# AdrianPerezHerrero/HDP-GPC

Measured on AMD Instinct MI355X. Metric: GP log-lik evals/sec (NxK batch, T-point segments), higher is better.
Workload: dtype f64; 1 GPU; BASELINE configs[1]: synthetic 2048 segments x 8 clusters, T=128, fp64, irregular segment grids (per-pair Gram + Cholesky + score); segments=2048, segments_per_gpu=2048, clusters=8, T=128

## Files before the change

hdpgpc_amd/csrc/hgp_pairs_acc.hip:

```cpp
#include <hip/hip_runtime.h>
#include <math.h>
#include <stdint.h>

#include "hgp_internal.hpp"
#include "tile_f64.hpp"

using namespace hgp;

namespace {

__host__ __device__ constexpr int ntl(int NB) { return NB * (NB - 1) / 2; }
__host__ __device__ constexpr int tl(int K, int Kp) { return K * (K - 1) / 2 + Kp; }

__global__ void k_acc_flags(double* scal, int K, double tol, int32_t* acc_list) {
  if (threadIdx.x != 0 || blockIdx.x != 0) return;
  int n = 0;
  for (int k = 0; k < K; ++k) {
    const double ck = scal[8 * k] * scal[8 * k + 6];
    const double bound = F64_EPS * ck * ck;
    const bool flag = (tol == 0.0) || (tol > 0.0 && !(bound <= tol));
    scal[8 * k + 7] = flag ? 1.0 : 0.0;
    if (flag) acc_list[1 + n++] = k;
  }
  acc_list[0] = n;
}

template <int NB>
__global__ __launch_bounds__(64) void k_acc_factor(double* A, int TP, const double* scal, int32_t* info) {
  __shared__ __attribute__((aligned(16))) double scr[DIAG_SCR];
  const int k = blockIdx.x, lane = threadIdx.x;
  if (scal[8 * k + 7] == 0.0) return;
  double* Ak = A + (size_t)k * TP * TP;
  d4 U[NB * (NB + 1) / 2];
  d4 R[NB];
  load_upper_only<NB>(U, Ak, TP, TP, lane);
  PivotAcc pa;
  pa.init();
  wave_factor<NB, 0>(U, R, scr, nullptr, nullptr, lane, pa, Ak, TP, TP);
  if (lane == 0 && info && pa.info != 0) info[k] = pa.info;
}

struct AccPrepArgs {
  const double* L;
  const double* S;
  const double* mean;
  const double* scal;
  int T, TP, NB;
  double* Lop;
  double* LTop;
  double* Dop;
  double* Sop;
  double* mu;
};

__global__ __launch_bounds__(256) void k_acc_prep(AccPrepArgs a) {
  const int k = blockIdx.x;
  if (a.scal[8 * k + 7] == 0.0) return;
  const int lane = threadIdx.x & 63, g = lane >> 4, c = lane & 15;
  const int wv = blockIdx.y * 4 + (threadIdx.x >> 6), nwv = gridDim.y * 4;
  const int NB = a.NB, TP = a.TP;
  const double* L = a.L + (size_t)k * TP * TP;
  const double* S = a.S + (size_t)k * TP * TP;
  const int nl = ntl(NB);
  double* Lop = a.Lop + (size_t)k * nl * 256;
  double* LTop = a.LTop + (size_t)k * nl * 256;
  double* Dop = a.Dop + (size_t)k * 4 * NB * 256;
  double* Sop = a.Sop + (size_t)k * NB * NB * 256;
  if (blockIdx.y == 0)
    for (int i = threadIdx.x; i < TP; i += 256) a.mu[(size_t)k * TP + i] = (i < a.T) ? a.mean[(size_t)k * a.T + i] : 0.0;
  const int items = nl + NB + NB * NB;
  for (int it = wv; it < items; it += nwv) {
    if (it < nl) {
      int Kb = 1;
      while (tl(Kb + 1, 0) <= it) ++Kb;
      const int Kp = it - tl(Kb, 0);
      d4 lo, lt;
#pragma unroll
      for (int s = 0; s < 4; ++s) {
        lo[s] = L[(size_t)(16 * Kb + c) * TP + 16 * Kp + 4 * s + g];
        lt[s] = L[(size_t)(16 * Kb + 4 * s + g) * TP + 16 * Kp + c];
      }
      *reinterpret_cast<d4*>(Lop + ((size_t)it * 64 + lane) * 4) = lo;
      *reinterpret_cast<d4*>(LTop + ((size_t)it * 64 + lane) * 4) = lt;
    } else if (it < nl + NB) {
      const int Kb = it - nl;
      const double* D = L + (size_t)(16 * Kb) * TP + 16 * Kb;
      d4 a1, a2, a1t, a2t;
#pragma unroll
      for (int r = 0; r < 4; ++r) {
        const double* B = D + (size_t)(4 * r) * TP + 4 * r;
        const double l00 = B[0], l10 = B[TP], l11 = B[TP + 1], l20 = B[2 * TP], l21 = B[2 * TP + 1], l22 = B[2 * TP + 2],
                     l30 = B[3 * (size_t)TP], l31 = B[3 * (size_t)TP + 1], l32 = B[3 * (size_t)TP + 2], l33 = B[3 * (size_t)TP + 3];
        double w[4][4];
#pragma unroll
        for (int i = 0; i < 4; ++i)
#pragma unroll
          for (int j = 0; j < 4; ++j) w[i][j] = 0.0;
        const double r0 = 1.0 / l00, r1 = 1.0 / l11, r2 = 1.0 / l22, r3 = 1.0 / l33;
        w[0][0] = r0;
        w[1][0] = -(l10 * w[0][0]) * r1;
        w[2][0] = -(l20 * w[0][0] + l21 * w[1][0]) * r2;
        w[3][0] = -(l30 * w[0][0] + l31 * w[1][0] + l32 * w[2][0]) * r3;
        w[1][1] = r1;
        w[2][1] = -(l21 * w[1][1]) * r2;
        w[3][1] = -(l31 * w[1][1] + l32 * w[2][1]) * r3;
        w[2][2] = r2;
        w[3][2] = -(l32 * w[2][2]) * r3;
        w[3][3] = r3;
        const int ci = c & 3;
        double wf = 0.0, wt = 0.0;
#pragma unroll
        for (int i = 0; i < 4; ++i)
#pragma unroll
          for (int j = 0; j < 4; ++j) {
            if (i == ci && j == g) wf = w[i][j];
            if (i == g && j == ci) wt = w[i][j];
          }
        const bool mine = (c >> 2) == r;
        a1[r] = mine ? wf : 0.0;
        a1t[r] = mine ? wt : 0.0;
        a2[r] = (c >= 4 * r + 4) ? D[(size_t)c * TP + 4 * r + g] : 0.0;
        a2t[r] = (c < 4 * r) ? D[(size_t)(4 * r + g) * TP + c] : 0.0;
      }
      *reinterpret_cast<d4*>(Dop + ((size_t)(0 * NB + Kb) * 64 + lane) * 4) = a1;
      *reinterpret_cast<d4*>(Dop + ((size_t)(1 * NB + Kb) * 64 + lane) * 4) = a2;
      *reinterpret_cast<d4*>(Dop + ((size_t)(2 * NB + Kb) * 64 + lane) * 4) = a1t;
      *reinterpret_cast<d4*>(Dop + ((size_t)(3 * NB + Kb) * 64 + lane) * 4) = a2t;
    } else {
      const int t = it - nl - NB, Kb = t / NB, Kp = t % NB;
      d4 so;
#pragma unroll
      for (int s = 0; s < 4; ++s) so[s] = S[(size_t)(16 * Kp + 4 * s + g) * TP + 16 * Kb + c];
      *reinterpret_cast<d4*>(Sop + ((size_t)t * 64 + lane) * 4) = so;
    }
  }
}

struct AccArgs {
  const double* x;
  const double* y;
  int N, Ts;
  const double* xb;
  int T;
  const double* scal;
  const double* mu;
  const double* Lop;
  const double* LTop;
  const double* Dop;
  const double* Sop;
  const int32_t* acc_list;
  const double* first_noise;
  const int32_t* sel;
  int K;
  double* out_quad;
  double* out_logdet;
  int32_t* out_info;
  double* sscr;
  double score_add;
  int score_on;
};

template <int NB>
struct AccLds {
  static constexpr int TP = 16 * NB;
  static constexpr size_t DOUBLES = (size_t)NB * 256  + 256  + 5 * TP  + DIAG_SCR + 32;
  static constexpr size_t BYTES = DOUBLES * sizeof(double) + 16 * sizeof(int);
};

__device__ __forceinline__ d4 ld4(const double* base, unsigned off) { return *reinterpret_cast<const d4*>(base + off); }

template <int NB>
__global__ __launch_bounds__(64 * CoopH<NB>::NW, (NB <= 8) ? 2 : 1) void k_pairs_acc(AccArgs a) {
  using H = CoopH<NB>;
  constexpr int NW = H::NW, TP = 16 * NB;
  extern __shared__ __attribute__((aligned(16))) double smem[];
  double* rowbuf = smem;
  double* Wbuf = rowbuf + NB * 256;
  double* dvec = Wbuf + 256;
  double* xs = dvec + TP;
  double* ys = xs + TP;
  double* xbs = ys + TP;
  double* mus = xbs + TP;
  double* scr = mus + TP;
  double* red = scr + DIAG_SCR;
  int* redi = reinterpret_cast<int*>(red + 32);
  const int tid = threadIdx.x, lane = tid & 63, g = lane >> 4, c = lane & 15;
  const int wave = __builtin_amdgcn_readfirstlane(tid >> 6);
  const int T = a.T, Ts = a.Ts;
  const int nflag = a.acc_list[0];
  if (nflag == 0) return;
  const long npairs = a.sel ? (long)a.N : (long)a.N * nflag;
  double* Ssc = a.sscr + (size_t)blockIdx.x * NB * NB * 256;

  for (long p = blockIdx.x; p < npairs; p += gridDim.x) {
    int n, kc;
    if (a.sel) {
      n = (int)p;
      kc = a.sel[n];
      if (a.scal[8 * kc + 7] == 0.0) continue;
    } else {
      n = (int)(p / nflag);
      kc = a.acc_list[1 + (int)(p % nflag)];
    }
    kc = __builtin_amdgcn_readfirstlane(kc);
    const double* sc = a.scal + 8 * kc;
    const double cc = sc[0], ell = sc[1], noise = sc[2];
    const bool iso = sc[3] != 0.0;
    const size_t oidx = a.sel ? (size_t)n : (size_t)n * a.K + kc;
    const double fn = a.first_noise ? a.first_noise[oidx] : 0.0;
    __syncthreads();
    for (int i = tid; i < TP; i += 64 * NW) {
      xs[i] = (i < Ts) ? a.x[(size_t)n * Ts + i] / ell : 1e150 * (double)(1 + i);
      ys[i] = (i < Ts) ? a.y[(size_t)n * Ts + i] : 0.0;
      xbs[i] = (i < T) ? a.xb[i] / ell : -1e150 * (double)(1 + i);
      mus[i] = a.mu[(size_t)kc * TP + i];
    }
    __syncthreads();
    const double* Lop = a.Lop + (size_t)kc * ntl(NB) * 256;
    const double* LTop = a.LTop + (size_t)kc * ntl(NB) * 256;
    const double* Dop = a.Dop + (size_t)kc * 4 * NB * 256;
    const double* Sop = a.Sop + (size_t)kc * NB * NB * 256;
    double* Sl = Ssc;

    double dsq = 0.0;
#pragma unroll
    for (int q = 0; q < 2; ++q) {
      const int J = (q == 0) ? wave : NB - 1 - wave;
      d4 X[NB];
#pragma unroll
      for (int K = 0; K < NB; ++K) {
        const unsigned l4 = (unsigned)launder(lane) * 4u;
        {
          const int ln = launder(lane);
          const double xj = xs[16 * J + (ln & 15)];
#pragma unroll
          for (int r = 0; r < 4; ++r) {
            const double u = xbs[16 * K + 4 * r + (ln >> 4)] - xj;
            X[K][r] = cc * exp(-0.5 * (u * u));
          }
        }
#pragma unroll
        for (int Kp = 0; Kp < K; ++Kp) {
          const d4 lo = ld4(Lop + tl(K, Kp) * 256, l4);
#pragma unroll
          for (int s = 0; s < 4; ++s) X[K] = mfma_sub(lo[s], X[Kp][s], X[K]);
        }
        const d4 a1 = ld4(Dop + (0 * NB + K) * 256, l4), a2 = ld4(Dop + (1 * NB + K) * 256, l4);
#pragma unroll
        for (int r = 0; r < 4; ++r) {
          d4 t = X[K];
          t[r] = 0.0;
          t = mfma(a1[r], X[K][r], t);
          X[K] = (r < 3) ? mfma_sub(a2[r], t[r], t) : t;
        }
      }
#pragma unroll
      for (int K = NB - 1; K >= 0; --K) {
        const unsigned l4 = (unsigned)launder(lane) * 4u;
#pragma unroll
        for (int Kp = NB - 1; Kp > K; --Kp) {
          const d4 lt = ld4(LTop + tl(Kp, K) * 256, l4);
#pragma unroll
          for (int s = 0; s < 4; ++s) X[K] = mfma_sub(lt[s], X[Kp][s], X[K]);
        }
        const d4 a1 = ld4(Dop + (2 * NB + K) * 256, l4), a2 = ld4(Dop + (3 * NB + K) * 256, l4);
#pragma unroll
        for (int r = 3; r >= 0; --r) {
          d4 t = X[K];
          t[r] = 0.0;
          t = mfma(a1[r], X[K][r], t);
          X[K] = (r > 0) ? mfma_sub(a2[r], t[r], t) : t;
        }
      }
      double pj = 0.0;
#pragma unroll
      for (int K = 0; K < NB; ++K) {
        const int ln = launder(lane);
        const unsigned l4 = (unsigned)ln * 4u;
#pragma unroll
        for (int r = 0; r < 4; ++r) pj = fma(X[K][r], mus[16 * K + 4 * r + (ln >> 4)], pj);
        *reinterpret_cast<d4*>(Sl + (K * NB + J) * 256 + l4) = X[K];
      }
      pj = xrow_sum(pj);
      if (g == 0) {
        const int j = 16 * J + c;
        const double d = ys[j] - pj;
        dvec[j] = d;
        dsq = fma(d, d, dsq);
      }
    }
    __syncthreads();

    if (iso) {
      dsq = wave_sum(dsq);
      if (lane == 0) red[wave] = dsq;
      __syncthreads();
      if (tid == 0) {
        const double v = sc[4] + fn;
        const double v2 = v + 1e-8 * fmax(fabs(v), F64_EPS);
        double tot_ = 0.0;
        for (int w_ = 0; w_ < NW; ++w_) tot_ += red[w_];
        a.out_quad[oidx] = a.score_on ? fma(-0.5, tot_ / v2, a.score_add) : (tot_ / v2);
        if (a.out_logdet) a.out_logdet[oidx] = (double)Ts * log(v2);
        if (a.out_info) a.out_info[oidx] = (v2 > 0.0) ? 0 : 1;
      }
      continue;
    }

    d4 U[H::NT];
#pragma unroll
    for (int q = 0; q < 2; ++q) {
      const int J = (q == 0) ? wave : NB - 1 - wave;
      const double xj = xs[16 * J + c];
#pragma unroll
      for (int I = 0; I < (q == 0 ? NW : NB); ++I) {
        const int ln = launder(lane);
        d4 kt = (d4){0.0, 0.0, 0.0, 0.0};
        if (I <= J) {
#pragma unroll
          for (int r = 0; r < 4; ++r) {
            const double u = xs[16 * I + (ln >> 4) + 4 * r] - xs[16 * J + (ln & 15)];
            kt[r] = cc * exp(-0.5 * (u * u));
          }
          if (I == J) {
#pragma unroll
            for (int r = 0; r < 4; ++r)
              if ((ln >> 4) + 4 * r == (ln & 15)) kt[r] = (16 * I + (ln & 15) < Ts) ? cc + noise : 1.0;
          }
          U[q == 0 ? H::slotA(I) : H::slotB(I)] = kt;
        }
      }
#pragma nounroll
      for (int K = 0; K < NB; ++K) {
        const unsigned l4 = (unsigned)launder(lane) * 4u;
        d4 Q;
#pragma unroll
        for (int r = 0; r < 4; ++r) {
          const double u = xbs[16 * K + 4 * r + g] - xj;
          Q[r] = -(cc * exp(-0.5 * (u * u)));
        }
#pragma unroll
        for (int Kp = 0; Kp < NB; ++Kp) {
          const d4 so = ld4(Sop + (K * NB + Kp) * 256, l4);
          const d4 sb = ld4(Sl + (Kp * NB + J) * 256, l4);
#pragma unroll
          for (int s = 0; s < 4; ++s) Q = mfma(so[s], sb[s], Q);
        }
#pragma unroll
        for (int I = 0; I < (q == 0 ? NW : NB); ++I) {
          if (I <= J) {
            const d4 sa = ld4(Sl + (K * NB + I) * 256, l4);
#pragma unroll
            for (int s = 0; s < 4; ++s)
              U[q == 0 ? H::slotA(I) : H::slotB(I)] = mfma(sa[s], Q[s], U[q == 0 ? H::slotA(I) : H::slotB(I)]);
          }
        }
      }
    }

    {
      const double sh = 1e-6 + fn;
      const double dm = cooph_diag_abs_mean<NB>(U, Ts, wave, lane, sh, red);
      cooph_add_diag<NB>(U, sh + 1e-8 * fmax(dm, F64_EPS), Ts, wave, lane);
    }
    PivotAcc pa;
    pa.init();
    double zq = cooph_factor<NB>(U, rowbuf, Wbuf, scr, wave, lane, pa, Ts, dvec);
    int info;
    const double ld = cooph_logdet_info<NB>(pa, wave, lane, red, redi, info);
    zq = wave_sum(zq);
    if (lane == 0) red[8 + wave] = zq;
    __syncthreads();
    if (tid == 0) {
      double tot_ = 0.0;
      for (int w_ = 0; w_ < NW; ++w_) tot_ += red[8 + w_];
      a.out_quad[oidx] = a.score_on ? fma(-0.5, tot_, a.score_add) : (tot_);
      if (a.out_logdet) a.out_logdet[oidx] = ld;
      if (a.out_info) a.out_info[oidx] = info;
    }
  }
}

template <int NB>
int launch_pairs_acc(const AccArgs& a, hipStream_t st) {
  const size_t lds = AccLds<NB>::BYTES;
  hipLaunchKernelGGL(k_pairs_acc<NB>, dim3(acc_grid_for(NB)), dim3(64 * CoopH<NB>::NW), lds, st, a);
  return launch_status();
}

}

size_t hgp_internal_acc_bytes(int TP, int K, size_t* sizes) {
  const int NB = TP / 16;
  size_t s[6];
  s[0] = (size_t)K * ntl(NB) * 256 * sizeof(double);
  s[1] = s[0];
  s[2] = (size_t)K * 4 * NB * 256 * sizeof(double);
  s[3] = (size_t)K * NB * NB * 256 * sizeof(double);
  s[4] = (size_t)K * TP * sizeof(double);
  s[5] = (size_t)acc_grid_for(NB) * NB * NB * 256 * sizeof(double);
  size_t tot = 0;
  for (int i = 0; i < 6; ++i) {
    if (sizes) sizes[i] = s[i];
    tot += (s[i] + 255) & ~(size_t)255;
  }
  return tot;
}

int hgp_internal_acc_prep(hgp_pairs_plan* p, const double* mean, hipStream_t st) {
  const int K = p->K, TP = p->TP, NB = p->NB;
  hipLaunchKernelGGL(k_acc_flags, dim3(1), dim3(64), 0, st, p->d_scal, K, p->acc_tol, p->d_acc_list);
  if (p->acc_tol < 0.0) return launch_status();
  if (NB <= 8)
    dispatch_nb_wave(TP, [&](auto nb) {
      hipLaunchKernelGGL(k_acc_factor<decltype(nb)::value>, dim3(K), dim3(64), 0, st, p->d_A, TP, p->d_scal, (int32_t*)nullptr);
    });
  AccPrepArgs a{p->d_A, p->d_S, mean, p->d_scal, p->T, TP, NB, p->d_Lop, p->d_LTop, p->d_Dop, p->d_Sop, p->d_mu};
  hipLaunchKernelGGL(k_acc_prep, dim3(K, 8), dim3(256), 0, st, a);
  return launch_status();
}

int hgp_internal_pairs_acc(const hgp_pairs_plan* p, const double* x, const double* y, int N, int Ts, const double* first_noise,
                           const int32_t* sel, double* out_quad, double* out_logdet, int32_t* out_info, hipStream_t st) {
  if (p->acc_tol < 0.0) return 0;
  AccArgs a{x, y, N, Ts, p->d_xb, p->T, p->d_scal, p->d_mu, p->d_Lop, p->d_LTop, p->d_Dop, p->d_Sop, p->d_acc_list,
            first_noise, sel, p->K, out_quad, out_logdet, out_info, p->d_sscr, -0.5 * (double)Ts * 1.8378770664093453, p->score_out};
  return dispatch_nb(p->NB, [&](auto nb) { return launch_pairs_acc<decltype(nb)::value>(a, st); });
}
```

hdpgpc_amd/csrc/hgp_plan.hip:

```cpp
#include <algorithm>
#include <new>

#include "hgp_internal.hpp"
#include "tile_f64.hpp"

using namespace hgp;

namespace {

struct PrepArgs {
  const double* xb;
  const double* mean;
  const double* Sigma;
  int T, TP, K;
  const double* theta;
  double* scal;
  double* A;
  double* S;
  double* xb_copy;
};

__global__ __launch_bounds__(256) void k_prep_build(PrepArgs a) {
  __shared__ double red[256];
  __shared__ int redi[256];
  const int k = blockIdx.x, tid = threadIdx.x;
  const int T = a.T, TP = a.TP;
  const double* Sg = a.Sigma + (size_t)k * T * T;
  const double c = a.theta[3 * k], ell = a.theta[3 * k + 1], noise = a.theta[3 * k + 2];
  double s_abs = 0.0, s_sgn = 0.0;
  for (int i = tid; i < T; i += 256) {
    double d = Sg[(size_t)i * T + i];
    s_abs += fabs(d);
    s_sgn += d;
  }
  red[tid] = s_abs;
  __syncthreads();
  for (int o = 128; o > 0; o >>= 1) {
    if (tid < o) red[tid] += red[tid + o];
    __syncthreads();
  }
  const double mean_abs = red[0] / T;
  __syncthreads();
  red[tid] = s_sgn;
  __syncthreads();
  for (int o = 128; o > 0; o >>= 1) {
    if (tid < o) red[tid] += red[tid + o];
    __syncthreads();
  }
  const double mS = red[0] / T;
  int bad = 0;
  for (int i = tid; i < T; i += 256) {
    double d = Sg[(size_t)i * T + i];
    if (!(fabs(d - mS) <= 1e-8 + 1e-5 * fabs(mS))) bad = 1;
  }
  redi[tid] = bad;
  __syncthreads();
  for (int o = 128; o > 0; o >>= 1) {
    if (tid < o) redi[tid] |= redi[tid + o];
    __syncthreads();
  }
  const double jit = 1e-4 * fmax(mean_abs, F64_EPS);
  if (tid == 0 && blockIdx.y == 0) {
    double* sc = a.scal + 8 * k;
    sc[0] = c;
    sc[1] = ell;
    sc[2] = noise;
    sc[3] = redi[0] ? 0.0 : 1.0;
    sc[4] = mS;
    sc[5] = jit;
    sc[6] = 0.0;
  }
  if (k == 0 && blockIdx.y == 0)
    for (int i = tid; i < TP; i += 256) a.xb_copy[i] = (i < T) ? a.xb[i] : 0.0;
  double* Ak = a.A + (size_t)k * TP * TP;
  double* Sk = a.S + (size_t)k * TP * TP;
  for (int idx = blockIdx.y * 256 + tid; idx < TP * TP; idx += gridDim.y * 256) {
    int i = idx / TP, j = idx % TP;
    double av, sv = 0.0;
    if (i < T && j < T) {
      double u = a.xb[i] / ell - a.xb[j] / ell;
      av = c * exp(-0.5 * (u * u));
      if (i == j) av += jit;
      sv = 0.5 * (Sg[(size_t)i * T + j] + Sg[(size_t)j * T + i]);
    } else {
      av = (i == j) ? 1.0 : 0.0;
    }
    Ak[idx] = av;
    Sk[idx] = sv;
  }
}

struct PrepFinalArgs {
  const double* Q;
  const double* Kinv;
  const double* mean;
  double* scal;
  int T, TP;
  double* Mp;
  double* ap;
  int interleave;
  int32_t* fb;
};

__global__ __launch_bounds__(256) void k_prep_final(PrepFinalArgs a) {
  const int k = blockIdx.x, tid = threadIdx.x;
  if (a.fb && k == 0 && blockIdx.y == 0 && tid == 0) {
    a.fb[0] = 0;
    a.fb[1 + PAIRS_FB_CAP] = 0;
  }
  const int T = a.T, TP = a.TP;
  const double c = a.scal[8 * k];
  const double* Q = a.Q + (size_t)k * TP * TP;
  const double* Ki = a.Kinv + (size_t)k * TP * TP;
  double* Mp = a.Mp + (size_t)k * TP * TP;
  __shared__ double tq[32][33], tk[32][33];
  const int NHh = (TP / 16) / 2, nt = TP / 32;
  const int tx = tid & 31, ty = tid >> 5;
  for (int t = blockIdx.y; t < nt * nt; t += gridDim.y) {
    const int bi = t / nt, bj = t % nt;
    __syncthreads();
#pragma unroll
    for (int r = 0; r < 4; ++r) {
      const int y = ty + 8 * r;
      tq[y][tx] = Q[(size_t)(32 * bj + y) * TP + 32 * bi + tx];
      tk[y][tx] = Ki[(size_t)(32 * bj + y) * TP + 32 * bi + tx];
    }
    __syncthreads();
#pragma unroll
    for (int r = 0; r < 4; ++r) {
      const int y = ty + 8 * r;
      const int i = 32 * bi + y, j = 32 * bj + tx;
      double v = 0.0;
      if (i < T && j < T)
        v = (c * c) * (0.5 * (Q[(size_t)i * TP + j] + tq[tx][y]) - 0.5 * (Ki[(size_t)i * TP + j] + tk[tx][y]));
      int jp = j;
      if (a.interleave) {
        const int hh = j / (16 * NHh), tl = (j / 16) % NHh, cc = j % 16;
        const int loc = (tl < 2 * (NHh / 2)) ? 32 * (tl / 2) + 2 * cc + (tl & 1) : 16 * (NHh - 1) + cc;
        jp = 16 * NHh * hh + loc;
      }
      Mp[(size_t)i * TP + jp] = v;
    }
  }
  const double* mu = a.mean + (size_t)k * T;
  __shared__ double red[256];
  double rmax = 0.0;
  for (int i = blockIdx.y * 256 + tid; i < TP; i += gridDim.y * 256) {
    double s = 0.0, rs = 0.0;
    if (i < T) {
#pragma unroll 8
      for (int j = 0; j < T; ++j) {
        const double kij = Ki[(size_t)j * TP + i];
        s = fma(kij, mu[j], s);
        rs += fabs(kij);
      }
    }
    a.ap[(size_t)k * TP + i] = c * s;
    rmax = fmax(rmax, rs);
  }
  red[tid] = rmax;
  __syncthreads();
  for (int o = 128; o > 0; o >>= 1) {
    if (tid < o) red[tid] = fmax(red[tid], red[tid + o]);
    __syncthreads();
  }
  if (tid == 0) atomicMax(reinterpret_cast<unsigned long long*>(a.scal + 8 * k + 6), (unsigned long long)__double_as_longlong(red[0]));
}

static int tp_for(int n) {
  if (n <= HGP_MAX_T_WAVE) return 16 * nb_for(n);
  return n <= 192 ? 192 : 256;
}

size_t plan_layout(hgp_pairs_plan* p, int T, int Ts_max, int K, char* base) {
  const size_t TP = (size_t)tp_for(std::max(T, Ts_max));
  const size_t mat = (size_t)K * TP * TP * sizeof(double);
  p->TP = (int)TP;
  p->NB = p->TP / 16;
  p->coop = p->TP > HGP_MAX_T_WAVE;
  size_t o = 0;
  auto take = [&](auto*& member, size_t bytes) {
    if (base) member = reinterpret_cast<std::remove_reference_t<decltype(member)>>(base + o);
    o += (bytes + 255) & ~(size_t)255;
  };
  take(p->d_theta, (size_t)K * 3 * sizeof(double));
  take(p->d_scal, (size_t)K * 8 * sizeof(double));
  take(p->d_A, mat);
  take(p->d_S, mat);
  take(p->d_Z, mat);
  take(p->d_Kinv, mat);
  take(p->d_P, mat);
  take(p->d_Q, mat);
  take(p->d_Mp, mat);
  take(p->d_ap, (size_t)K * TP * sizeof(double));
  take(p->d_perm, (size_t)K * sizeof(int32_t));
  take(p->d_xb, TP * sizeof(double));
  if (p->coop) {
    const size_t nb = (size_t)p->NB;
    const size_t cap = (nb >= 12) ? 48 : (nb == 8 ? 24 : 16);
    const size_t over = nb * nb > cap ? nb * nb - cap : 0;
    p->nscr = over ? (nb >= 12 ? 512 : 1024) : 0;
    p->escr_stride = (long)(over * 256);
    take(p->d_escr, (size_t)p->nscr * over * 256 * sizeof(double));
    take(p->d_eflags, ((size_t)p->nscr + 1) * sizeof(int32_t));
  }
  size_t sz[6];
  hgp_internal_acc_bytes((int)TP, K, sz);
  take(p->d_Lop, sz[0]);
  take(p->d_LTop, sz[1]);
  take(p->d_Dop, sz[2]);
  take(p->d_Sop, sz[3]);
  take(p->d_mu, sz[4]);
  take(p->d_sscr, sz[5]);
  take(p->d_acc_list, (size_t)(K + 1) * sizeof(int32_t));
  take(p->d_fb, (size_t)(PAIRS_FB_CAP + 2) * sizeof(int32_t));
  return o;
}

}

#ifdef HGP_STAMPS
unsigned long long* hgp_internal_stamp_dev = nullptr;
#endif

extern "C" {

size_t hgp_pairs_plan_device_bytes(int T, int Ts_max, int K) {
  if (T <= 0 || Ts_max <= 0 || K <= 0) return 0;
  hgp_pairs_plan sizing;
  return plan_layout(&sizing, T, Ts_max, K, nullptr);
}

int hgp_pairs_plan_create(hgp_pairs_plan** plan, int T, int Ts_max, int K, const double* theta_host, void* dev_buf,
                          size_t dev_bytes) {
  if (!plan || !theta_host || !dev_buf || T <= 0 || Ts_max <= 0 || K <= 0) return -1;
  if (T > HGP_MAX_T_COOP || Ts_max > HGP_MAX_T_COOP) return -2;
  if (dev_bytes < hgp_pairs_plan_device_bytes(T, Ts_max, K)) return -1;
  for (int k = 0; k < K; ++k)
    if (!(theta_host[3 * k] > 0.0) || !(theta_host[3 * k + 1] > 0.0)) return -1;
  hgp_pairs_plan* p = new (std::nothrow) hgp_pairs_plan();
  if (!p) return -1;
  p->T = T;
  p->K = K;
  p->theta.assign(theta_host, theta_host + 3 * (size_t)K);
  p->perm.resize(K);
  for (int k = 0; k < K; ++k) p->perm[k] = k;
  std::stable_sort(p->perm.begin(), p->perm.end(),
                   [&](int a, int b) { return p->theta[3 * a + 1] < p->theta[3 * b + 1]; });
  for (int i = 0; i < K;) {
    int j = i;
    double ell = p->theta[3 * p->perm[i] + 1];
    while (j < K && p->theta[3 * p->perm[j] + 1] == ell) ++j;
    p->grp_beg.push_back(i);
    p->grp_end.push_back(j);
    p->grp_ell.push_back(ell);
    i = j;
  }
  plan_layout(p, T, Ts_max, K, (char*)dev_buf);
  if (hipMemset(p->d_fb, 0, (size_t)(PAIRS_FB_CAP + 2) * sizeof(int32_t)) != hipSuccess) {
    delete p;
    return 1000 + (int)hipGetLastError();
  }
  if (p->coop && hipMemset(p->d_eflags, 0, (p->nscr + 1) * sizeof(int32_t)) != hipSuccess) {
    delete p;
    return 1000 + (int)hipGetLastError();
  }
  if (hipMemcpy(p->d_theta, p->theta.data(), sizeof(double) * 3 * K, hipMemcpyHostToDevice) != hipSuccess ||
      hipMemcpy(p->d_perm, p->perm.data(), sizeof(int32_t) * K, hipMemcpyHostToDevice) != hipSuccess) {
    delete p;
    return 1000 + (int)hipGetLastError();
  }
  *plan = p;
  return 0;
}

void hgp_pairs_plan_destroy(hgp_pairs_plan* plan) { delete plan; }

const double* hgp_pairs_plan_scalars(const hgp_pairs_plan* plan) { return plan ? plan->d_scal : nullptr; }

int hgp_pairs_plan_update(hgp_pairs_plan* p, const double* x_basis, const double* mean, const double* Sigma,
                          int32_t* info, void* stream) {
  if (!p || !x_basis || !mean || !Sigma) return -1;
  hipStream_t st = (hipStream_t)stream;
  const int K = p->K, T = p->T, TP = p->TP;
  PrepArgs pa{x_basis, mean, Sigma, T, TP, K, p->d_theta, p->d_scal, p->d_A, p->d_S, p->d_xb};
  hipLaunchKernelGGL(k_prep_build, dim3(K, 8), dim3(256), 0, st, pa);
  PotrfArgs fa{p->d_A, TP, K, 0.0, 0.0, p->d_Z, nullptr, info};
  fa.inv_info = 1;
  fa.symmetric = 1;
  if (int rc = hgp_internal_chol_inverse(fa, p->NB, st)) return rc;
  const long sm = (long)TP * TP;
  GemmArgs g1{p->d_Z, p->d_Z, p->d_Kinv, TP, TP, TP, TP, TP, TP, sm, sm, sm, 1.0, 0.0, 1, 0};
  GemmArgs g2{p->d_S, p->d_Kinv, p->d_P, TP, TP, TP, TP, TP, TP, sm, sm, sm, 1.0, 0.0, 0, 0};
  GemmArgs g3{p->d_Kinv, p->d_P, p->d_Q, TP, TP, TP, TP, TP, TP, sm, sm, sm, 1.0, 0.0, 0, 0};
  hgp_internal_gemm(g1, K, st);
  hgp_internal_gemm(g2, K, st);
  hgp_internal_gemm(g3, K, st);
  PrepFinalArgs fin{p->d_Q, p->d_Kinv, mean, p->d_scal, T, TP, p->d_Mp, p->d_ap, p->coop ? 0 : 1, p->d_fb};
  hipLaunchKernelGGL(k_prep_final, dim3(K, 8), dim3(256), 0, st, fin);
  if (p->d_eflags && p->nscr > 0 && hipMemsetAsync(p->d_eflags, 0, (p->nscr + 1) * sizeof(int32_t), st) != hipSuccess) return launch_status();
  int rc = hgp_internal_acc_prep(p, mean, st);
  return rc ? rc : launch_status();
}

int hgp_pairs_plan_set_accuracy(hgp_pairs_plan* p, double tol) {
  if (!p || tol != tol) return -1;
  p->acc_tol = tol;
  return 0;
}

int hgp_pairs_plan_set_score_output(hgp_pairs_plan* p, int on) {
  if (!p) return -1;
  p->score_out = on ? 1 : 0;
  return 0;
}

int hgp_loglik_pairs_f64(const hgp_pairs_plan* p, const double* x, const double* y, int N, int Ts,
                         const double* first_noise, const int32_t* sel, double* out_quad, double* out_logdet,
                         int32_t* out_info, void* stream) {
  if (N == 0) return 0;
  if (!p || !x || !y || !out_quad || N < 0 || Ts <= 0) return -1;
  if (Ts > HGP_MAX_T_COOP) return -2;
  if (Ts > p->TP) return -2;
  hipStream_t st = (hipStream_t)stream;
  int rc = 0;
  if (p->coop && p->d_eflags && p->nscr > 0 &&
      hipMemsetAsync(p->d_eflags, 0, (p->nscr + 1) * sizeof(int32_t), st) != hipSuccess)
    return launch_status();
  for (size_t gi = 0; gi < p->grp_beg.size() && rc == 0; ++gi) {
    PairsArgs a{x, y, N, Ts, p->d_xb, p->T, p->d_Mp, p->d_ap, p->d_scal, p->d_perm, p->grp_beg[gi], p->grp_end[gi],
                p->grp_ell[gi], first_noise, sel,
#ifdef HGP_STAMPS
                hgp_internal_stamp_dev,
#endif
                p->K, out_quad, out_logdet, out_info, p->d_escr, p->d_eflags, p->nscr, p->escr_stride,
                env_on("HGP_PAIRS_GENERIC") ? 1 : 0, -0.5 * (double)Ts * 1.8378770664093453, p->score_out, p->d_fb};
    rc = hgp_internal_pairs_fast(a, p->NB, p->coop, st);
  }
  if (rc == 0) rc = hgp_internal_pairs_acc(p, x, y, N, Ts, first_noise, sel, out_quad, out_logdet, out_info, st);
  return rc;
}

#ifdef HGP_STAMPS
int hgp_debug_stamps(unsigned long long* out8_host) {
  if (!hgp_internal_stamp_dev) {
    if (hipMalloc(&hgp_internal_stamp_dev, 128) != hipSuccess) return 1;
    (void)hipMemset(hgp_internal_stamp_dev, 0, 128);
  }
  if (hipMemcpy(out8_host, hgp_internal_stamp_dev, 128, hipMemcpyDeviceToHost) != hipSuccess) return 1;
  (void)hipMemset(hgp_internal_stamp_dev, 0, 128);
  return 0;
}
#endif

}
```

Before: 15.43 million evals/s.

## Fuse plan-update GEMMs and accuracy setup into fewer custom kernels

Replaces the two generic batched GEMMs (S·Kinv, Kinv·P) and the final M'/a' kernel with two templated MFMA tile kernels for the non-cooperative path. These compute P, then Q tiles with the symmetrised M' and interleaved column layout, and fold the a' reduction into the first kernel. The accuracy flag, Cholesky factor and operand packing are merged into a single setup kernel. Gram/Sigma construction is retiled over a 3-D grid. The aim is fewer kernel launches and fewer global round-trips during plan updates, at the cost of more specialised code paths and intra-block fences that the correctness of the fused factor-then-pack step relies on.

Result: no change. 15.57 million evals/s (median of 6 runs) (+0.9%).

```diff
diff --git a/hdpgpc_amd/csrc/hgp_pairs_acc.hip b/hdpgpc_amd/csrc/hgp_pairs_acc.hip
--- a/hdpgpc_amd/csrc/hgp_pairs_acc.hip
+++ b/hdpgpc_amd/csrc/hgp_pairs_acc.hip
@@ -12,32 +12,25 @@
 __host__ __device__ constexpr int ntl(int NB) { return NB * (NB - 1) / 2; }
 __host__ __device__ constexpr int tl(int K, int Kp) { return K * (K - 1) / 2 + Kp; }
 
+__device__ __forceinline__ bool acc_flag_of(const double* scal, int k, double tol) {
+  const double ck = scal[8 * k] * scal[8 * k + 6];
+  const double bound = F64_EPS * ck * ck;
+  return (tol == 0.0) || (tol > 0.0 && !(bound <= tol));
+}
+
+__device__ __forceinline__ void acc_write_flags(double* scal, int K, double tol, int32_t* acc_list) {
+  int n = 0;
+  for (int k = 0; k < K; ++k) {
+    const bool flag = acc_flag_of(scal, k, tol);
+    scal[8 * k + 7] = flag ? 1.0 : 0.0;
+    if (flag) acc_list[1 + n++] = k;
+  }
+  acc_list[0] = n;
+}
+
 __global__ void k_acc_flags(double* scal, int K, double tol, int32_t* acc_list) {
   if (threadIdx.x != 0 || blockIdx.x != 0) return;
-  int n = 0;
-  for (int k = 0; k < K; ++k) {
-    const double ck = scal[8 * k] * scal[8 * k + 6];
-    const double bound = F64_EPS * ck * ck;
-    const bool flag = (tol == 0.0) || (tol > 0.0 && !(bound <= tol));
-    scal[8 * k + 7] = flag ? 1.0 : 0.0;
-    if (flag) acc_list[1 + n++] = k;
-  }
-  acc_list[0] = n;
-}
-
-template <int NB>
-__global__ __launch_bounds__(64) void k_acc_factor(double* A, int TP, const double* scal, int32_t* info) {
-  __shared__ __attribute__((aligned(16))) double scr[DIAG_SCR];
-  const int k = blockIdx.x, lane = threadIdx.x;
-  if (scal[8 * k + 7] == 0.0) return;
-  double* Ak = A + (size_t)k * TP * TP;
-  d4 U[NB * (NB + 1) / 2];
-  d4 R[NB];
-  load_upper_only<NB>(U, Ak, TP, TP, lane);
-  PivotAcc pa;
-  pa.init();
-  wave_factor<NB, 0>(U, R, scr, nullptr, nullptr, lane, pa, Ak, TP, TP);
-  if (lane == 0 && info && pa.info != 0) info[k] = pa.info;
+  acc_write_flags(scal, K, tol, acc_list);
 }
 
 struct AccPrepArgs {
@@ -53,11 +46,8 @@
   double* mu;
 };
 
-__global__ __launch_bounds__(256) void k_acc_prep(AccPrepArgs a) {
-  const int k = blockIdx.x;
-  if (a.scal[8 * k + 7] == 0.0) return;
+__device__ __forceinline__ void acc_pack(const AccPrepArgs& a, int k, int it0, int it1, int wv, int nwv) {
   const int lane = threadIdx.x & 63, g = lane >> 4, c = lane & 15;
-  const int wv = blockIdx.y * 4 + (threadIdx.x >> 6), nwv = gridDim.y * 4;
   const int NB = a.NB, TP = a.TP;
   const double* L = a.L + (size_t)k * TP * TP;
   const double* S = a.S + (size_t)k * TP * TP;
@@ -66,10 +56,7 @@
   double* LTop = a.LTop + (size_t)k * nl * 256;
   double* Dop = a.Dop + (size_t)k * 4 * NB * 256;
   double* Sop = a.Sop + (size_t)k * NB * NB * 256;
-  if (blockIdx.y == 0)
-    for (int i = threadIdx.x; i < TP; i += 256) a.mu[(size_t)k * TP + i] = (i < a.T) ? a.mean[(size_t)k * a.T + i] : 0.0;
-  const int items = nl + NB + NB * NB;
-  for (int it = wv; it < items; it += nwv) {
+  for (int it = it0 + wv; it < it1; it += nwv) {
     if (it < nl) {
       int Kb = 1;
       while (tl(Kb + 1, 0) <= it) ++Kb;
@@ -134,6 +121,47 @@
       *reinterpret_cast<d4*>(Sop + ((size_t)t * 64 + lane) * 4) = so;
     }
   }
+}
+
+__device__ __forceinline__ void acc_copy_mean(const AccPrepArgs& a, int k) {
+  for (int i = threadIdx.x; i < a.TP; i += 256) a.mu[(size_t)k * a.TP + i] = (i < a.T) ? a.mean[(size_t)k * a.T + i] : 0.0;
+}
+
+__global__ __launch_bounds__(256) void k_acc_prep(AccPrepArgs a) {
+  const int k = blockIdx.x;
+  if (a.scal[8 * k + 7] == 0.0) return;
+  if (blockIdx.y == 0) acc_copy_mean(a, k);
+  acc_pack(a, k, 0, ntl(a.NB) + a.NB + a.NB * a.NB, blockIdx.y * 4 + (threadIdx.x >> 6), gridDim.y * 4);
+}
+
+constexpr int ACC_SBLK = 7;
+
+template <int NB>
+__global__ __launch_bounds__(256) void k_acc_setup(AccPrepArgs a, double* A, double* scal, int K, double tol, int32_t* acc_list) {
+  __shared__ __attribute__((aligned(16))) double scr[DIAG_SCR];
+  const int k = blockIdx.x;
+  if (k == 0 && blockIdx.y == 0 && threadIdx.x == 0) acc_write_flags(scal, K, tol, acc_list);
+  if (!acc_flag_of(a.scal, k, tol)) return;
+  const int nl = ntl(NB), wave = threadIdx.x >> 6;
+  if (blockIdx.y != 0) {
+    acc_pack(a, k, nl + NB, nl + NB + NB * NB, ((int)blockIdx.y - 1) * 4 + wave, ((int)gridDim.y - 1) * 4);
+    return;
+  }
+  acc_copy_mean(a, k);
+  if (wave == 0) {
+    const int lane = threadIdx.x;
+    double* Ak = A + (size_t)k * a.TP * a.TP;
+    d4 U[NB * (NB + 1) / 2];
+    d4 R[NB];
+    load_upper_only<NB>(U, Ak, a.TP, a.TP, lane);
+    PivotAcc pa;
+    pa.init();
+    wave_factor<NB, 0>(U, R, scr, nullptr, nullptr, lane, pa, Ak, a.TP, a.TP);
+    __threadfence();
+  }
+  __syncthreads();
+  __threadfence();
+  acc_pack(a, k, 0, nl + NB, wave, 4);
 }
 
 struct AccArgs {
@@ -409,13 +437,16 @@
 
 int hgp_internal_acc_prep(hgp_pairs_plan* p, const double* mean, hipStream_t st) {
   const int K = p->K, TP = p->TP, NB = p->NB;
+  AccPrepArgs a{p->d_A, p->d_S, mean, p->d_scal, p->T, TP, NB, p->d_Lop, p->d_LTop, p->d_Dop, p->d_Sop, p->d_mu};
+  if (NB <= 8) {
+    dispatch_nb_wave(TP, [&](auto nb) {
+      hipLaunchKernelGGL(k_acc_setup<decltype(nb)::value>, dim3(K, 1 + ACC_SBLK), dim3(256), 0, st, a, p->d_A, p->d_scal, K,
+                         p->acc_tol, p->d_acc_list);
+    });
+    return launch_status();
+  }
   hipLaunchKernelGGL(k_acc_flags, dim3(1), dim3(64), 0, st, p->d_scal, K, p->acc_tol, p->d_acc_list);
   if (p->acc_tol < 0.0) return launch_status();
-  if (NB <= 8)
-    dispatch_nb_wave(TP, [&](auto nb) {
-      hipLaunchKernelGGL(k_acc_factor<decltype(nb)::value>, dim3(K), dim3(64), 0, st, p->d_A, TP, p->d_scal, (int32_t*)nullptr);
-    });
-  AccPrepArgs a{p->d_A, p->d_S, mean, p->d_scal, p->T, TP, NB, p->d_Lop, p->d_LTop, p->d_Dop, p->d_Sop, p->d_mu};
   hipLaunchKernelGGL(k_acc_prep, dim3(K, 8), dim3(256), 0, st, a);
   return launch_status();
 }
diff --git a/hdpgpc_amd/csrc/hgp_plan.hip b/hdpgpc_amd/csrc/hgp_plan.hip
--- a/hdpgpc_amd/csrc/hgp_plan.hip
+++ b/hdpgpc_amd/csrc/hgp_plan.hip
@@ -60,7 +60,8 @@
     __syncthreads();
   }
   const double jit = 1e-4 * fmax(mean_abs, F64_EPS);
-  if (tid == 0 && blockIdx.y == 0) {
+  const bool first = blockIdx.y == 0 && blockIdx.z == 0;
+  if (tid == 0 && first) {
     double* sc = a.scal + 8 * k;
     sc[0] = c;
     sc[1] = ell;
@@ -70,23 +71,27 @@
     sc[5] = jit;
     sc[6] = 0.0;
   }
-  if (k == 0 && blockIdx.y == 0)
+  if (k == 0 && first)
     for (int i = tid; i < TP; i += 256) a.xb_copy[i] = (i < T) ? a.xb[i] : 0.0;
   double* Ak = a.A + (size_t)k * TP * TP;
   double* Sk = a.S + (size_t)k * TP * TP;
-  for (int idx = blockIdx.y * 256 + tid; idx < TP * TP; idx += gridDim.y * 256) {
-    int i = idx / TP, j = idx % TP;
+  const int i = 16 * (int)blockIdx.y + (tid >> 4);
+  const double ui = (i < T) ? a.xb[i] / ell : 0.0;
+#pragma unroll
+  for (int m = 0; m < 4; ++m) {
+    const int j = 64 * (int)blockIdx.z + 16 * m + (tid & 15);
+    if (j >= TP) break;
     double av, sv = 0.0;
     if (i < T && j < T) {
-      double u = a.xb[i] / ell - a.xb[j] / ell;
+      double u = ui - a.xb[j] / ell;
       av = c * exp(-0.5 * (u * u));
       if (i == j) av += jit;
       sv = 0.5 * (Sg[(size_t)i * T + j] + Sg[(size_t)j * T + i]);
     } else {
       av = (i == j) ? 1.0 : 0.0;
     }
-    Ak[idx] = av;
-    Sk[idx] = sv;
+    Ak[(size_t)i * TP + j] = av;
+    Sk[(size_t)i * TP + j] = sv;
   }
 }
 
@@ -98,9 +103,18 @@
   int T, TP;
   double* Mp;
   double* ap;
-  int interleave;
   int32_t* fb;
 };
+
+__device__ __forceinline__ double mprime_entry(double c, double q, double qt, double ki, double kit) {
+  return (c * c) * (0.5 * (q + qt) - 0.5 * (ki + kit));
+}
+
+__device__ __forceinline__ int mprime_col(int j, int NHh) {
+  const int hh = j / (16 * NHh), tl = (j / 16) % NHh, cc = j % 16;
+  const int loc = (tl < 2 * (NHh / 2)) ? 32 * (tl / 2) + 2 * cc + (tl & 1) : 16 * (NHh - 1) + cc;
+  return 16 * NHh * hh + loc;
+}
 
 __global__ __launch_bounds__(256) void k_prep_final(PrepFinalArgs a) {
   const int k = blockIdx.x, tid = threadIdx.x;
@@ -114,7 +128,7 @@
   const double* Ki = a.Kinv + (size_t)k * TP * TP;
   double* Mp = a.Mp + (size_t)k * TP * TP;
   __shared__ double tq[32][33], tk[32][33];
-  const int NHh = (TP / 16) / 2, nt = TP / 32;
+  const int nt = TP / 32;
   const int tx = tid & 31, ty = tid >> 5;
   for (int t = blockIdx.y; t < nt * nt; t += gridDim.y) {
     const int bi = t / nt, bj = t % nt;
@@ -132,14 +146,8 @@
       const int i = 32 * bi + y, j = 32 * bj + tx;
       double v = 0.0;
       if (i < T && j < T)
-        v = (c * c) * (0.5 * (Q[(size_t)i * TP + j] + tq[tx][y]) - 0.5 * (Ki[(size_t)i * TP + j] + tk[tx][y]));
-      int jp = j;
-      if (a.interleave) {
-        const int hh = j / (16 * NHh), tl = (j / 16) % NHh, cc = j % 16;
-        const int loc = (tl < 2 * (NHh / 2)) ? 32 * (tl / 2) + 2 * cc + (tl & 1) : 16 * (NHh - 1) + cc;
-        jp = 16 * NHh * hh + loc;
-      }
-      Mp[(size_t)i * TP + jp] = v;
+        v = mprime_entry(c, Q[(size_t)i * TP + j], tq[tx][y], Ki[(size_t)i * TP + j], tk[tx][y]);
+      Mp[(size_t)i * TP + j] = v;
     }
   }
   const double* mu = a.mean + (size_t)k * T;
@@ -165,6 +173,109 @@
     __syncthreads();
   }
   if (tid == 0) atomicMax(reinterpret_cast<unsigned long long*>(a.scal + 8 * k + 6), (unsigned long long)__double_as_longlong(red[0]));
+}
+
+template <int NB>
+__device__ __forceinline__ d4 tile_product(const double* __restrict__ A, const double* __restrict__ B, int ti, int tj, int lane) {
+  constexpr int TP = 16 * NB, NK = 4 * NB;
+  const int g = lane >> 4, c = lane & 15;
+  const double* Ar = A + (size_t)(16 * ti + c) * TP + g;
+  const double* Bc = B + (size_t)g * TP + 16 * tj + c;
+  double av[NK], bv[NK];
+#pragma unroll
+  for (int u = 0; u < NK; ++u) {
+    av[u] = Ar[4 * u];
+    bv[u] = Bc[(size_t)(4 * u) * TP];
+  }
+  d4 acc = (d4){0.0, 0.0, 0.0, 0.0};
+#pragma unroll
+  for (int u = 0; u < NK; ++u) acc = mfma(av[u], bv[u], acc);
+  return acc;
+}
+
+struct PlanFuseArgs {
+  const double* S;
+  const double* Kinv;
+  double* P;
+  const double* mean;
+  double* scal;
+  int T;
+  double* Mp;
+  double* ap;
+  int32_t* fb;
+};
+
+template <int NB>
+__global__ __launch_bounds__(256) void k_plan_p(PlanFuseArgs a) {
+  constexpr int TP = 16 * NB;
+  __shared__ double kt[TP][33];
+  __shared__ double mus[TP];
+  __shared__ double red[32];
+  const int k = blockIdx.y, tid = threadIdx.x;
+  const double* Ki = a.Kinv + (size_t)k * TP * TP;
+  if (blockIdx.x < NB * NB / 4) {
+    const int tile = blockIdx.x * 4 + (tid >> 6), lane = tid & 63;
+    const int ti = tile / NB, tj = tile % NB;
+    const d4 acc = tile_product<NB>(a.S + (size_t)k * TP * TP, Ki, ti, tj, lane);
+    double* P = a.P + (size_t)k * TP * TP;
+#pragma unroll
+    for (int r = 0; r < 4; ++r) P[(size_t)(16 * ti + (lane >> 4) + 4 * r) * TP + 16 * tj + (lane & 15)] = acc[r];
+    return;
+  }
+  const int T = a.T, i0 = 32 * ((int)blockIdx.x - NB * NB / 4);
+  for (int e = tid; e < 32 * T; e += 256) kt[e >> 5][e & 31] = Ki[(size_t)(e >> 5) * TP + i0 + (e & 31)];
+  for (int j = tid; j < T; j += 256) mus[j] = a.mean[(size_t)k * T + j];
+  __syncthreads();
+  if (tid < 32) {
+    const int i = i0 + tid;
+    double s = 0.0, rs = 0.0;
+    if (i < T) {
+#pragma unroll 8
+      for (int j = 0; j < T; ++j) {
+        const double kij = kt[j][tid];
+        s = fma(kij, mus[j], s);
+        rs += fabs(kij);
+      }
+    }
+    a.ap[(size_t)k * TP + i] = a.scal[8 * k] * s;
+    red[tid] = rs;
+  }
+  __syncthreads();
+  if (tid == 0) {
+    double rmax = 0.0;
+    for (int t = 0; t < 32; ++t) rmax = fmax(rmax, red[t]);
+    atomicMax(reinterpret_cast<unsigned long long*>(a.scal + 8 * k + 6), (unsigned long long)__double_as_longlong(rmax));
+  }
+}
+
+template <int NB>
+__global__ __launch_bounds__(256) void k_plan_m(PlanFuseArgs a) {
+  constexpr int TP = 16 * NB;
+  __shared__ double tr[4][16][17];
+  const int k = blockIdx.y, tid = threadIdx.x, wave = tid >> 6, lane = tid & 63;
+  if (blockIdx.x == 0 && k == 0 && tid == 0) {
+    a.fb[0] = 0;
+    a.fb[1 + PAIRS_FB_CAP] = 0;
+  }
+  const int g = lane >> 4, cidx = lane & 15;
+  const int tile = blockIdx.x * 4 + wave, ti = tile / NB, tj = tile % NB;
+  const double* Ki = a.Kinv + (size_t)k * TP * TP;
+  const double* P = a.P + (size_t)k * TP * TP;
+  const d4 q = tile_product<NB>(Ki, P, ti, tj, lane);
+  const d4 qm = (ti == tj) ? q : tile_product<NB>(Ki, P, tj, ti, lane);
+#pragma unroll
+  for (int r = 0; r < 4; ++r) tr[wave][g + 4 * r][cidx] = qm[r];
+  __syncthreads();
+  const double c = a.scal[8 * k];
+  double* Mp = a.Mp + (size_t)k * TP * TP;
+  const int j = 16 * tj + cidx;
+#pragma unroll
+  for (int r = 0; r < 4; ++r) {
+    const int i = 16 * ti + g + 4 * r;
+    double v = 0.0;
+    if (i < a.T && j < a.T) v = mprime_entry(c, q[r], tr[wave][cidx][g + 4 * r], Ki[(size_t)i * TP + j], Ki[(size_t)j * TP + i]);
+    Mp[(size_t)i * TP + mprime_col(j, NB / 2)] = v;
+  }
 }
 
 static int tp_for(int n) {
@@ -284,20 +395,29 @@
   hipStream_t st = (hipStream_t)stream;
   const int K = p->K, T = p->T, TP = p->TP;
   PrepArgs pa{x_basis, mean, Sigma, T, TP, K, p->d_theta, p->d_scal, p->d_A, p->d_S, p->d_xb};
-  hipLaunchKernelGGL(k_prep_build, dim3(K, 8), dim3(256), 0, st, pa);
+  hipLaunchKernelGGL(k_prep_build, dim3(K, TP / 16, (TP + 63) / 64), dim3(256), 0, st, pa);
   PotrfArgs fa{p->d_A, TP, K, 0.0, 0.0, p->d_Z, nullptr, info};
   fa.inv_info = 1;
   fa.symmetric = 1;
   if (int rc = hgp_internal_chol_inverse(fa, p->NB, st)) return rc;
   const long sm = (long)TP * TP;
   GemmArgs g1{p->d_Z, p->d_Z, p->d_Kinv, TP, TP, TP, TP, TP, TP, sm, sm, sm, 1.0, 0.0, 1, 0};
-  GemmArgs g2{p->d_S, p->d_Kinv, p->d_P, TP, TP, TP, TP, TP, TP, sm, sm, sm, 1.0, 0.0, 0, 0};
-  GemmArgs g3{p->d_Kinv, p->d_P, p->d_Q, TP, TP, TP, TP, TP, TP, sm, sm, sm, 1.0, 0.0, 0, 0};
   hgp_internal_gemm(g1, K, st);
-  hgp_internal_gemm(g2, K, st);
-  hgp_internal_gemm(g3, K, st);
-  PrepFinalArgs fin{p->d_Q, p->d_Kinv, mean, p->d_scal, T, TP, p->d_Mp, p->d_ap, p->coop ? 0 : 1, p->d_fb};
-  hipLaunchKernelGGL(k_prep_final, dim3(K, 8), dim3(256), 0, st, fin);
+  if (!p->coop) {
+    PlanFuseArgs fu{p->d_S, p->d_Kinv, p->d_P, mean, p->d_scal, T, p->d_Mp, p->d_ap, p->d_fb};
+    dispatch_nb_wave(TP, [&](auto nb) {
+      constexpr int NB = decltype(nb)::value;
+      hipLaunchKernelGGL(k_plan_p<NB>, dim3(NB * NB / 4 + NB / 2, K), dim3(256), 0, st, fu);
+      hipLaunchKernelGGL(k_plan_m<NB>, dim3(NB * NB / 4, K), dim3(256), 0, st, fu);
+    });
+  } else {
+    GemmArgs g2{p->d_S, p->d_Kinv, p->d_P, TP, TP, TP, TP, TP, TP, sm, sm, sm, 1.0, 0.0, 0, 0};
+    GemmArgs g3{p->d_Kinv, p->d_P, p->d_Q, TP, TP, TP, TP, TP, TP, sm, sm, sm, 1.0, 0.0, 0, 0};
+    hgp_internal_gemm(g2, K, st);
+    hgp_internal_gemm(g3, K, st);
+    PrepFinalArgs fin{p->d_Q, p->d_Kinv, mean, p->d_scal, T, TP, p->d_Mp, p->d_ap, p->d_fb};
+    hipLaunchKernelGGL(k_prep_final, dim3(K, 8), dim3(256), 0, st, fin);
+  }
   if (p->d_eflags && p->nscr > 0 && hipMemsetAsync(p->d_eflags, 0, (p->nscr + 1) * sizeof(int32_t), st) != hipSuccess) return launch_status();
   int rc = hgp_internal_acc_prep(p, mean, st);
   return rc ? rc : launch_status();
```
